# vincentjzy/OpenCorr

Hardware: AMD Instinct MI355X
Metric: converged POIs/sec (FFTCC+ICGN2D1, 33x33 subset) (higher is better)
Workload: dtype f32

## Files before the change

opencorr_amd/csrc/fftcc2d_fused.hip:

```cpp
#include "dic2d_device.h"
#include "fft_device.h"
#include "oc_kernels.h"
#include "host/fftcc_plan.h"

namespace ochip {

namespace {

using namespace fftdev;

constexpr int FN = ochip_host::kFftcc2dFusedSide;
constexpr int FP = FN + 1;
constexpr int FWAVE_LDS = FN * FP;
#ifndef OC_FFTCC2D_X2
#define OC_FFTCC2D_X2 1
#endif
#if !OC_FFTCC2D_X2
#ifndef OC_FFTCC2D_WAVES
#define OC_FFTCC2D_WAVES 4
#endif
constexpr int kFusedWaves = OC_FFTCC2D_WAVES;

template <bool INV>
__device__ __forceinline__ void fft32_line(const c2* line, int step, int h, c2 (&v)[16]) {
#pragma clang fp contract(fast)
    const float sgn = h ? -1.f : 1.f;
#pragma unroll
    for (int n = 0; n < 16; n++) {
        const c2 x0 = line[n * step], x1 = line[(n + 16) * step];
        const c2 d = x0 + sgn * x1;
        const float c = h ? kCos32[n] : 1.f, s = h ? kSin32[n] : 0.f;
        v[n] = (n == 0) ? d : cmul_tw<INV>(d, c, s);
    }
    fft16<INV>(v);
}
#endif

}

#if !OC_FFTCC2D_X2
__global__ __launch_bounds__(64 * kFusedWaves) void fftcc2d_fused32_kernel(Fftcc2dParams P, float* __restrict__ pois,
                                                                           int stride_f, unsigned long long count,
                                                                           int xcd_chunk) {
    __shared__ c2 lds[kFusedWaves * FWAVE_LDS];
    const int lane = threadIdx.x & (kWave - 1);
    const int wave = __builtin_amdgcn_readfirstlane(threadIdx.x >> 6);
    unsigned long long grp = blockIdx.x;
    if (xcd_chunk > 0) grp = (unsigned long long)(blockIdx.x & 7u) * xcd_chunk + (blockIdx.x >> 3);
    const unsigned long long idx = grp * kFusedWaves + wave;
    if (idx >= count) return;
    c2* buf = lds + wave * FWAVE_LDS;
    float* poi = pois + idx * (unsigned long long)stride_f;
    const float px = poi[poi2d::X], py = poi[poi2d::Y];
    const float gu = poi[poi2d::U], gv = poi[poi2d::V];
    const int rx = FN / 2, ry = FN / 2, width = P.width, height = P.height;
    constexpr int M = FN * FN;

    if ((int)px < rx || (int)px >= width - rx || (int)py < ry || (int)py >= height - ry || (int)(px + gu) < rx ||
        (int)(px + gu) >= width - rx || (int)(py + gv) < ry || (int)(py + gv) >= height - ry)
        return;

    float rn, tn;
    {
        const __amdgpu_buffer_rsrc_t r_ref = make_rsrc(P.ref), r_tar = make_rsrc(P.tar);
        float a[16], b[16];
        float rsum = 0.f, tsum = 0.f;
#pragma unroll
        for (int k = 0; k < 16; k++) {
            const int s = lane + kWave * k;
            const int r = s >> 5, c = s & 31;
            const float rxp = px + c - rx, ryp = py + r - ry;
            a[k] = buf_f32(r_ref, (__umul24((unsigned)(int)ryp, (unsigned)width) + (unsigned)(int)rxp) << 2, 0);
            const float txp = rxp + gu, typ = ryp + gv;
            b[k] = buf_f32(r_tar, (__umul24((unsigned)(int)typ, (unsigned)width) + (unsigned)(int)txp) << 2, 0);
        }
#pragma unroll
        for (int k = 0; k < 16; k++) {
            rsum += a[k];
            tsum += b[k];
        }
        const float rmean = wave_allreduce_sum(rsum) / M;
        const float tmean = wave_allreduce_sum(tsum) / M;
        rn = 0.f;
        tn = 0.f;
#pragma unroll
        for (int k = 0; k < 16; k++) {
            const int s = lane + kWave * k;
            const float x = a[k] - rmean, y = b[k] - tmean;
            rn += x * x;
            tn += y * y;
            buf[(s >> 5) * FP + (s & 31)] = mkc(x, y);
        }
        rn = wave_allreduce_sum(rn);
        tn = wave_allreduce_sum(tn);
    }
    __builtin_amdgcn_wave_barrier();

    const int line = lane & 31, h = lane >> 5;
    c2 v[16];
    fft32_line<false>(buf + line * FP, 1, h, v);
    __builtin_amdgcn_wave_barrier();
#pragma unroll
    for (int k = 0; k < 16; k++) buf[line * FP + 2 * k + h] = v[bitrev4(k)];
    __builtin_amdgcn_wave_barrier();
    fft32_line<false>(buf + line, FP, h, v);
    __builtin_amdgcn_wave_barrier();
#pragma unroll
    for (int k = 0; k < 16; k++) buf[(2 * k + h) * FP + line] = v[bitrev4(k)];
    __builtin_amdgcn_wave_barrier();
    {
        const int mx = (FN - line) & (FN - 1);
        c2 zm[16];
#pragma unroll
        for (int k = 0; k < 16; k++) zm[k] = buf[((FN - (2 * k + h)) & (FN - 1)) * FP + mx];
        __builtin_amdgcn_wave_barrier();
#pragma unroll
        for (int k = 0; k < 16; k++) {
            const c2 z = v[bitrev4(k)];
            const float rr = 0.5f * (z.x + zm[k].x), ri = 0.5f * (z.y - zm[k].y);
            const float tr = 0.5f * (z.y + zm[k].y), ti = -0.5f * (z.x - zm[k].x);
            buf[(2 * k + h) * FP + line] = mkc((rr * tr) + (ri * ti), (rr * ti) - (ri * tr));
        }
    }
    __builtin_amdgcn_wave_barrier();
    fft32_line<true>(buf + line * FP, 1, h, v);
    __builtin_amdgcn_wave_barrier();
#pragma unroll
    for (int k = 0; k < 16; k++) buf[line * FP + 2 * k + h] = v[bitrev4(k)];
    __builtin_amdgcn_wave_barrier();
    fft32_line<true>(buf + line, FP, h, v);

    float best = -2.f;
    int bidx = 0;
#pragma unroll
    for (int k = 0; k < 16; k++) {
        const float val = v[bitrev4(k)].x;
        if (val > best) { best = val; bidx = (2 * k + h) * FN + line; }
    }
#pragma unroll
    for (int off = 1; off < kWave; off <<= 1) {
        const float ov = __shfl_xor(best, off, kWave);
        const int oi = __shfl_xor(bidx, off, kWave);
        if (ov > best || (ov == best && oi < bidx)) { best = ov; bidx = oi; }
    }
    if (lane == 0) {
        int du = bidx % FN, dv = bidx / FN;
        if (du > rx) du -= FN;
        if (dv > ry) dv -= FN;
        poi[poi2d::U] = (float)du + gu;
        poi[poi2d::V] = (float)dv + gv;
        poi[poi2d::U0] = gu;
        poi[poi2d::V0] = gv;
        poi[poi2d::ZNCC] = best / (sqrtf(rn * tn) * M);
    }
}
#endif

#ifndef OC_FFTCC2D_X2_WAVES
#define OC_FFTCC2D_X2_WAVES 1
#endif
#ifndef OC_FFTCC2D_X2_SPLIT
#define OC_FFTCC2D_X2_SPLIT 1
#endif
#ifndef OC_FFTCC2D_X2_OCC
#define OC_FFTCC2D_X2_OCC (OC_FFTCC2D_X2_SPLIT ? 4 : 2)
#endif
constexpr int kX2Waves = OC_FFTCC2D_X2_WAVES;

__device__ __forceinline__ float half_wave_sum(float v) {
#pragma unroll
    for (int off = 1; off < 32; off <<= 1) v += __shfl_xor(v, off, kWave);
    return v;
}

template <bool FAST_ROWS, bool REAL_LAST>
__global__ __launch_bounds__(64 * kX2Waves, OC_FFTCC2D_X2_OCC) void fftcc2d_fused32x2_kernel(Fftcc2dParams P, float* __restrict__ pois, int stride_f,
                                                                         unsigned long long count, int xcd_chunk) {
    __shared__ c2 lds[kX2Waves * 2 * FWAVE_LDS / (OC_FFTCC2D_X2_SPLIT ? 2 : 1)];
    const int lane = threadIdx.x & (kWave - 1);
    const int wave = __builtin_amdgcn_readfirstlane(threadIdx.x >> 6);
    const int q = lane >> 5, l = lane & 31;
    unsigned long long grp = blockIdx.x;
    if (xcd_chunk > 0) grp = (unsigned long long)(blockIdx.x & 7u) * xcd_chunk + (blockIdx.x >> 3);
    const unsigned long long idx = (grp * kX2Waves + wave) * 2 + q;
    if (idx >= count) return;
    c2* tile = lds + (wave * 2 + q) * (FWAVE_LDS / (OC_FFTCC2D_X2_SPLIT ? 2 : 1));
    float* poi = pois + idx * (unsigned long long)stride_f;
    const float px = poi[poi2d::X], py = poi[poi2d::Y];
    const float gu = poi[poi2d::U], gv = poi[poi2d::V];
    const int rx = FN / 2, ry = FN / 2, width = P.width, height = P.height;
    constexpr int M = FN * FN;
    if ((int)px < rx || (int)px >= width - rx || (int)py < ry || (int)py >= height - ry || (int)(px + gu) < rx ||
        (int)(px + gu) >= width - rx || (int)(py + gv) < ry || (int)(py + gv) >= height - ry)
        return;

    c2 v[FN];
    float rn, tn;
    {
        const __amdgpu_buffer_rsrc_t r_ref = make_rsrc(P.ref), r_tar = make_rsrc(P.tar);
        const float rxp = px + l - rx, txp = rxp + gu;
        const bool integral = px == (float)(int)px && py == (float)(int)py && gu == (float)(int)gu && gv == (float)(int)gv;
        if (FAST_ROWS && __builtin_amdgcn_ballot_w64(!integral) == 0) {
            const float ry0 = py - ry, ty0 = ry0 + gv;
            const unsigned ref0 = (__umul24((unsigned)(int)ry0, (unsigned)width) + (unsigned)(int)rxp) << 2;
            const unsigned tar0 = (__umul24((unsigned)(int)ty0, (unsigned)width) + (unsigned)(int)txp) << 2;
            const unsigned pitch = (unsigned)width << 2;
#pragma unroll
            for (int k = 0; k < FN; k++) v[k] = mkc(buf_f32(r_ref, ref0, k * pitch), buf_f32(r_tar, tar0, k * pitch));
        } else {
#pragma unroll
            for (int k = 0; k < FN; k++) {
                const float ryp = py + k - ry, typ = ryp + gv;
                const float a = buf_f32(r_ref, (__umul24((unsigned)(int)ryp, (unsigned)width) + (unsigned)(int)rxp) << 2, 0);
                const float b = buf_f32(r_tar, (__umul24((unsigned)(int)typ, (unsigned)width) + (unsigned)(int)txp) << 2, 0);
                v[k] = mkc(a, b);
            }
        }
        float rsum = 0.f, tsum = 0.f;
#pragma unroll
        for (int k = 0; k < FN; k++) {
            rsum += v[k].x;
            tsum += v[k].y;
        }
        const c2 mean = mkc(half_wave_sum(rsum) / M, half_wave_sum(tsum) / M);
        rn = 0.f;
        tn = 0.f;
#pragma unroll
        for (int k = 0; k < FN; k++) {
            v[k] = v[k] - mean;
            rn += v[k].x * v[k].x;
            tn += v[k].y * v[k].y;
        }
        rn = half_wave_sum(rn);
        tn = half_wave_sum(tn);
        asm volatile("" : "+v"(rn), "+v"(tn));
    }
    fft32<false>(v);
#if OC_FFTCC2D_X2_SPLIT
    float* __restrict__ ft = reinterpret_cast<float*>(tile);
#define OC_X2_TRANSPOSE(WRITE_IDX, READ_IDX)                                                   \
    _Pragma("unroll") for (int k = 0; k < FN; k++) ft[WRITE_IDX] = v[bitrev5(k)].x;            \
    __builtin_amdgcn_wave_barrier();                                                           \
    _Pragma("unroll") for (int k = 0; k < FN; k++) v[k].x = ft[READ_IDX];                      \
    __builtin_amdgcn_wave_barrier();                                                           \
    _Pragma("unroll") for (int k = 0; k < FN; k++) ft[WRITE_IDX] = v[bitrev5(k)].y;            \
    __builtin_amdgcn_wave_barrier();                                                           \
    _Pragma("unroll") for (int k = 0; k < FN; k++) v[k].y = ft[READ_IDX];                      \
    __builtin_amdgcn_wave_barrier();
#else
#define OC_X2_TRANSPOSE(WRITE_IDX, READ_IDX)                                                   \
    _Pragma("unroll") for (int k = 0; k < FN; k++) tile[WRITE_IDX] = v[bitrev5(k)];            \
    __builtin_amdgcn_wave_barrier();                                                           \
    _Pragma("unroll") for (int k = 0; k < FN; k++) v[k] = tile[READ_IDX];                      \
    __builtin_amdgcn_wave_barrier();
#endif
    OC_X2_TRANSPOSE(k * FP + l, l * FP + k)
    fft32<false>(v);
    {
        const int mrow = ((FN - l) & (FN - 1)) * FP;
        auto product = [](c2 z, c2 zm) {
            const float rr = z.x + zm.x, ri = z.y - zm.y;
            const float tr = z.y + zm.y, ti = zm.x - z.x;
            return mkc((rr * tr) + (ri * ti), (rr * ti) - (ri * tr));
        };
#if OC_FFTCC2D_X2_SPLIT
        float zmx[FN];
#pragma unroll
        for (int k = 0; k < FN; k++) ft[l * FP + k] = v[bitrev5(k)].x;
        __builtin_amdgcn_wave_barrier();
#pragma unroll
        for (int k = 0; k < FN; k++) zmx[k] = ft[mrow + ((FN - k) & (FN - 1))];
        __builtin_amdgcn_wave_barrier();
#pragma unroll
        for (int k = 0; k < FN; k++) ft[l * FP + k] = v[bitrev5(k)].y;
        __builtin_amdgcn_wave_barrier();
#pragma unroll
        for (int k = 0; k < FN; k++) v[bitrev5(k)] = product(v[bitrev5(k)], mkc(zmx[k], ft[mrow + ((FN - k) & (FN - 1))]));
        __builtin_amdgcn_wave_barrier();
#else
#pragma unroll
        for (int k = 0; k < FN; k++) tile[l * FP + k] = v[bitrev5(k)];
        __builtin_amdgcn_wave_barrier();
#pragma unroll
        for (int k = 0; k < FN; k++) v[bitrev5(k)] = product(v[bitrev5(k)], tile[mrow + ((FN - k) & (FN - 1))]);
        __builtin_amdgcn_wave_barrier();
#endif
    }
    c2 u[FN];
#pragma unroll
    for (int k = 0; k < FN; k++) u[k] = v[bitrev5(k)];
    fft32<true>(u);
#pragma unroll
    for (int k = 0; k < FN; k++) v[k] = u[k];
    float best = -2.f;
    int bidx = 0;
    if constexpr (REAL_LAST) {
#if OC_FFTCC2D_X2_SPLIT
#pragma unroll
        for (int k = 0; k < FN; k++) ft[l * FP + k] = v[bitrev5(k)].x;
        __builtin_amdgcn_wave_barrier();
#pragma unroll
        for (int k = 0; k <= FN / 2; k++) v[k].x = ft[k * FP + l];
        __builtin_amdgcn_wave_barrier();
#pragma unroll
        for (int k = 0; k < FN; k++) ft[l * FP + k] = v[bitrev5(k)].y;
        __builtin_amdgcn_wave_barrier();
#pragma unroll
        for (int k = 0; k <= FN / 2; k++) v[k].y = ft[k * FP + l];
#else
#pragma unroll
        for (int k = 0; k < FN; k++) tile[l * FP + k] = v[bitrev5(k)];
        __builtin_amdgcn_wave_barrier();
#pragma unroll
        for (int k = 0; k <= FN / 2; k++) v[k] = tile[k * FP + l];
#endif
        c2 z[FN / 2];
        ifft32_hermitian(v, z);
        static_for<0, FN>([&](auto rc) {
            constexpr int r = decltype(rc)::value;
            constexpr int pos = fft_pos(FN / 2, r >> 1);
            const float val = (r & 1) ? z[pos].y : z[pos].x;
            if (val > best) { best = val; bidx = r * FN + l; }
        });
    } else {
        OC_X2_TRANSPOSE(l * FP + k, k * FP + l)
#pragma unroll
        for (int k = 0; k < FN; k++) u[k] = v[k];
        fft32<true>(u);
#pragma unroll
        for (int r = 0; r < FN; r++) {
            const float val = u[bitrev5(r)].x;
            if (val > best) { best = val; bidx = r * FN + l; }
        }
    }
#undef OC_X2_TRANSPOSE
#pragma unroll
    for (int off = 1; off < 32; off <<= 1) {
        const float ov = __shfl_xor(best, off, kWave);
        const int oi = __shfl_xor(bidx, off, kWave);
        if (ov > best || (ov == best && oi < bidx)) { best = ov; bidx = oi; }
    }
    if (l == 0) {
        if (rn == 0.f || tn == 0.f) {
            best = 0.f;
            bidx = 0;
        }
        int du = bidx % FN, dv = bidx / FN;
        if (du > rx) du -= FN;
        if (dv > ry) dv -= FN;
        poi[poi2d::U] = (float)du + gu;
        poi[poi2d::V] = (float)dv + gv;
        poi[poi2d::U0] = gu;
        poi[poi2d::V0] = gv;
        poi[poi2d::ZNCC] = (0.25f * best) / (sqrtf(rn * tn) * M);
    }
}

hipError_t launch_fftcc2d_fused(const Fftcc2dParams& p, float* pois, int stride_f, size_t count, bool xcd,
                                hipStream_t stream, int body) {
    if (count == 0) return hipSuccess;
    if (ochip_host::fftcc2d_kernel(p.rx, p.ry, 1) != ochip_host::Fftcc2dKernel::Fused32) return hipErrorInvalidValue;
    (void)hipGetLastError();
#if OC_FFTCC2D_X2
    {
        const size_t groups = (count + 2 * kX2Waves - 1) / (2 * kX2Waves);
        const int chunk = xcd ? (int)((groups + 7) / 8) : 0;
        const size_t grid = xcd ? (size_t)chunk * 8 : groups;
        auto kern = body == 3 ? fftcc2d_fused32x2_kernel<false, false>
                    : body == 4 ? fftcc2d_fused32x2_kernel<true, false>
                    : body == 5 ? fftcc2d_fused32x2_kernel<false, true>
                                : fftcc2d_fused32x2_kernel<true, true>;
        hipLaunchKernelGGL(kern, dim3((unsigned)grid), dim3(64 * kX2Waves), 0, stream, p, pois, stride_f,
                           (unsigned long long)count, chunk);
        return hipGetLastError();
    }
#else
    const size_t groups = (count + kFusedWaves - 1) / kFusedWaves;
    const int chunk = xcd ? (int)((groups + 7) / 8) : 0;
    const size_t grid = xcd ? (size_t)chunk * 8 : groups;
    hipLaunchKernelGGL(fftcc2d_fused32_kernel, dim3((unsigned)grid), dim3(64 * kFusedWaves), 0, stream, p, pois, stride_f,
                       (unsigned long long)count, chunk);
    return hipGetLastError();
#endif
}

}
```

Before: 85.50 million.

## Pair two waves per block to split real-FFT spectrum product work

Adds a paired-wave body for the real-last FFTCC path: two waves (four subsets) share LDS, and one alternating wave computes the Hermitian cross-spectrum product and inverse row FFTs for all four subsets while the other waits. Block size becomes 128 threads for this path and the launch grid is recomputed accordingly. The aim is to halve the redundant product/unpack work and improve balance, at the cost of block-level syncthreads, extra LDS, and idle time for the non-producer wave.

```diff
diff --git a/opencorr_amd/csrc/fftcc2d_fused.hip b/opencorr_amd/csrc/fftcc2d_fused.hip
--- a/opencorr_amd/csrc/fftcc2d_fused.hip
+++ b/opencorr_amd/csrc/fftcc2d_fused.hip
@@ -174,8 +174,8 @@
 }
 
 template <bool FAST_ROWS, bool REAL_LAST>
-__global__ __launch_bounds__(64 * kX2Waves, OC_FFTCC2D_X2_OCC) void fftcc2d_fused32x2_kernel(Fftcc2dParams P, float* __restrict__ pois, int stride_f,
-                                                                         unsigned long long count, int xcd_chunk) {
+__device__ __forceinline__ void fused32x2_wave_body(const Fftcc2dParams& P, float* __restrict__ pois, int stride_f,
+                                                    unsigned long long count, int xcd_chunk) {
     __shared__ c2 lds[kX2Waves * 2 * FWAVE_LDS / (OC_FFTCC2D_X2_SPLIT ? 2 : 1)];
     const int lane = threadIdx.x & (kWave - 1);
     const int wave = __builtin_amdgcn_readfirstlane(threadIdx.x >> 6);
@@ -356,6 +356,239 @@
     }
 }
 
+#ifndef OC_FFTCC2D_X2_PAIR
+#define OC_FFTCC2D_X2_PAIR (OC_FFTCC2D_X2_SPLIT && OC_FFTCC2D_X2_WAVES == 1)
+#endif
+#if OC_FFTCC2D_X2_PAIR
+constexpr int kPairTile = FN * FP + 16;
+constexpr int kPairLds = 4 * kPairTile + 4 * 2 * FN;
+
+template <bool FAST_ROWS>
+__device__ __forceinline__ void fused32x2_pair_body(const Fftcc2dParams& P, float* __restrict__ pois, int stride_f,
+                                                    unsigned long long count, int xcd_chunk) {
+    __shared__ __attribute__((aligned(16))) float lds[kPairLds];
+    const int lane = threadIdx.x & (kWave - 1);
+    const int wave = __builtin_amdgcn_readfirstlane(threadIdx.x >> 6);
+    const int q = lane >> 5, l = lane & 31;
+    unsigned long long grp = blockIdx.x;
+    if (xcd_chunk > 0) grp = (unsigned long long)(blockIdx.x & 7u) * xcd_chunk + (blockIdx.x >> 3);
+    const bool prod = wave == (int)((blockIdx.x >> 3) & 1u);
+    const unsigned long long idx = (grp * 2 + wave) * 2 + q;
+    float* ft = lds + (wave * 2 + q) * kPairTile;
+    float* poi = pois + idx * (unsigned long long)stride_f;
+    const int rx = FN / 2, ry = FN / 2, width = P.width, height = P.height;
+    constexpr int M = FN * FN;
+    float px = 0.f, py = 0.f, gu = 0.f, gv = 0.f;
+    const bool in_queue = idx < count;
+    if (in_queue) {
+        px = poi[poi2d::X];
+        py = poi[poi2d::Y];
+        gu = poi[poi2d::U];
+        gv = poi[poi2d::V];
+    }
+    const bool live = in_queue && !((int)px < rx || (int)px >= width - rx || (int)py < ry || (int)py >= height - ry ||
+                                    (int)(px + gu) < rx || (int)(px + gu) >= width - rx || (int)(py + gv) < ry ||
+                                    (int)(py + gv) >= height - ry);
+    const unsigned long long live_mask = __builtin_amdgcn_ballot_w64(live);
+    auto half_waves = [](float x, float& h0, float& h1) {
+        h0 = __int_as_float(__builtin_amdgcn_readlane(__float_as_int(x), 0));
+        h1 = __int_as_float(__builtin_amdgcn_readlane(__float_as_int(x), 32));
+        asm volatile("" : "+s"(h0), "+s"(h1));
+    };
+    unsigned long long idx0 = (grp * 2 + wave) * 2;
+    asm volatile("" : "+s"(idx0));
+    float gu0, gu1, gv0, gv1, rn0, rn1, tn0, tn1;
+    half_waves(gu, gu0, gu1);
+    half_waves(gv, gv0, gv1);
+
+    c2 v[FN];
+    float rn, tn;
+    {
+        if (!live) {
+            float zero;
+            asm volatile("v_mov_b32 %0, 0" : "=v"(zero));
+#pragma unroll
+            for (int k = 0; k < FN; k++) v[k] = mkc(zero, zero);
+        } else {
+            const __amdgpu_buffer_rsrc_t r_ref = make_rsrc(P.ref), r_tar = make_rsrc(P.tar);
+            const float rxp = px + l - rx, txp = rxp + gu;
+            const bool integral = px == (float)(int)px && py == (float)(int)py && gu == (float)(int)gu && gv == (float)(int)gv;
+            if (FAST_ROWS && __builtin_amdgcn_ballot_w64(!integral) == 0) {
+                const float ry0 = py - ry, ty0 = ry0 + gv;
+                const unsigned ref0 = (__umul24((unsigned)(int)ry0, (unsigned)width) + (unsigned)(int)rxp) << 2;
+                const unsigned tar0 = (__umul24((unsigned)(int)ty0, (unsigned)width) + (unsigned)(int)txp) << 2;
+                const unsigned pitch = (unsigned)width << 2;
+#pragma unroll
+                for (int k = 0; k < FN; k++) v[k] = mkc(buf_f32(r_ref, ref0, k * pitch), buf_f32(r_tar, tar0, k * pitch));
+            } else {
+#pragma unroll
+                for (int k = 0; k < FN; k++) {
+                    const float ryp = py + k - ry, typ = ryp + gv;
+                    const float a = buf_f32(r_ref, (__umul24((unsigned)(int)ryp, (unsigned)width) + (unsigned)(int)rxp) << 2, 0);
+                    const float b = buf_f32(r_tar, (__umul24((unsigned)(int)typ, (unsigned)width) + (unsigned)(int)txp) << 2, 0);
+                    v[k] = mkc(a, b);
+                }
+            }
+        }
+        float rsum = 0.f, tsum = 0.f;
+#pragma unroll
+        for (int k = 0; k < FN; k++) {
+            rsum += v[k].x;
+            tsum += v[k].y;
+        }
+        const c2 mean = mkc(half_wave_sum(rsum) / M, half_wave_sum(tsum) / M);
+        rn = 0.f;
+        tn = 0.f;
+#pragma unroll
+        for (int k = 0; k < FN; k++) {
+            v[k] = v[k] - mean;
+            rn += v[k].x * v[k].x;
+            tn += v[k].y * v[k].y;
+        }
+        half_waves(half_wave_sum(rn), rn0, rn1);
+        half_waves(half_wave_sum(tn), tn0, tn1);
+    }
+    fft32<false>(v);
+#pragma unroll
+    for (int k = 0; k < FN; k++) ft[k * FP + l] = v[bitrev5(k)].x;
+    __builtin_amdgcn_wave_barrier();
+#pragma unroll
+    for (int k = 0; k < FN; k++) v[k].x = ft[l * FP + k];
+    __builtin_amdgcn_wave_barrier();
+#pragma unroll
+    for (int k = 0; k < FN; k++) ft[k * FP + l] = v[bitrev5(k)].y;
+    __builtin_amdgcn_wave_barrier();
+#pragma unroll
+    for (int k = 0; k < FN; k++) v[k].y = ft[l * FP + k];
+    __builtin_amdgcn_wave_barrier();
+    fft32<false>(v);
+
+    const int p = lane >> 4, j = lane & 15;
+    float* pt = lds + p * kPairTile;
+    c2* spare = reinterpret_cast<c2*>(lds + 4 * kPairTile) + p * FN;
+    const int zrow = j * FP, mrow = ((FN - j) & (FN - 1)) * FP;
+    auto product = [](c2 z, c2 zm) {
+        const float rr = z.x + zm.x, ri = z.y - zm.y;
+        const float tr = z.y + zm.y, ti = zm.x - z.x;
+        return mkc((rr * tr) + (ri * ti), (rr * ti) - (ri * tr));
+    };
+    c2 za[FN / 2], zma[FN / 2], ea[4];
+    const int jm = (FN / 2 - j) & (FN / 2 - 1);
+#pragma unroll
+    for (int k = 0; k < FN / 2; k++) {
+        ft[l * FP + 2 * k] = v[bitrev5(k)].x;
+        ft[l * FP + 2 * k + 1] = v[bitrev5(k)].y;
+    }
+#pragma unroll
+    for (int k = FN / 2; k < FN; k++) asm volatile("" : "+v"(v[bitrev5(k)]));
+    __syncthreads();
+    auto at = [&](int row, int k) { return mkc(pt[row + 2 * k], pt[row + 2 * k + 1]); };
+    if (prod) {
+#pragma unroll
+        for (int k = 0; k < FN / 2; k++) {
+            za[k] = at(zrow, k);
+            zma[k] = at(mrow, k);
+        }
+        ea[0] = at(0, j);
+        ea[1] = at((FN / 2) * FP, j);
+        ea[2] = at(0, jm);
+        ea[3] = at((FN / 2) * FP, jm);
+    }
+    __syncthreads();
+#pragma unroll
+    for (int k = 0; k < FN / 2; k++) {
+        ft[l * FP + 2 * k] = v[bitrev5(FN / 2 + k)].x;
+        ft[l * FP + 2 * k + 1] = v[bitrev5(FN / 2 + k)].y;
+    }
+    __syncthreads();
+    if (prod) {
+        c2 u[FN];
+        u[0] = product(za[0], zma[0]);
+        u[FN / 2] = product(at(zrow, 0), at(mrow, 0));
+#pragma unroll
+        for (int k = 1; k < FN / 2; k++) {
+            u[k] = product(za[k], at(mrow, FN / 2 - k));
+            u[FN / 2 + k] = product(at(zrow, k), zma[FN / 2 - k]);
+        }
+        {
+            const c2 eb[4] = {at(0, j), at((FN / 2) * FP, j), at(0, jm), at((FN / 2) * FP, jm)};
+            const bool self = j == 0;
+#pragma unroll
+            for (int t = 0; t < 2; t++) {
+                const c2 z0 = t ? eb[0] : ea[0], z16 = t ? eb[1] : ea[1];
+                const c2 o0 = t ? ea[2] : eb[2], o16 = t ? ea[3] : eb[3];
+                const c2 m0 = mkc(self ? z0.x : o0.x, self ? z0.y : o0.y), m16 = mkc(self ? z16.x : o16.x, self ? z16.y : o16.y);
+                const c2 d0 = product(z0, m0), d16 = product(z16, m16);
+                spare[j + 16 * t] = mkc(d0.x - d16.y, d0.y + d16.x);
+            }
+        }
+        __builtin_amdgcn_wave_barrier();
+        if (j == 0) {
+#pragma unroll
+            for (int k = 0; k < FN; k++) u[k] = spare[k];
+        }
+        fft32<true>(u);
+#pragma unroll
+        for (int c = 0; c < FN; c++) pt[zrow + c] = u[bitrev5(c)].x;
+#pragma unroll
+        for (int c = 0; c < FN; c++) pt[(FN / 2) * FP + zrow + c] = u[bitrev5(c)].y;
+    }
+    __syncthreads();
+
+#pragma unroll
+    for (int k = 0; k <= FN / 2; k++) v[k].x = ft[k * FP + l];
+    v[0].y = 0.f;
+    v[FN / 2].y = 0.f;
+#pragma unroll
+    for (int k = 1; k < FN / 2; k++) v[k].y = ft[(FN / 2 + k) * FP + l];
+    c2 z[FN / 2];
+    ifft32_hermitian(v, z);
+    float best = -2.f;
+    int bidx = 0;
+    static_for<0, FN>([&](auto rc) {
+        constexpr int r = decltype(rc)::value;
+        constexpr int pos = fft_pos(FN / 2, r >> 1);
+        const float val = (r & 1) ? z[pos].y : z[pos].x;
+        if (val > best) { best = val; bidx = r * FN + l; }
+    });
+#pragma unroll
+    for (int off = 1; off < 32; off <<= 1) {
+        const float ov = __shfl_xor(best, off, kWave);
+        const int oi = __shfl_xor(bidx, off, kWave);
+        if (ov > best || (ov == best && oi < bidx)) { best = ov; bidx = oi; }
+    }
+    if (l == 0 && ((live_mask >> lane) & 1ull)) {
+        const float wu = q ? gu1 : gu0, wv = q ? gv1 : gv0, wrn = q ? rn1 : rn0, wtn = q ? tn1 : tn0;
+        float* rec = pois + (idx0 + q) * (unsigned long long)stride_f;
+        if (wrn == 0.f || wtn == 0.f) {
+            best = 0.f;
+            bidx = 0;
+        }
+        int du = bidx % FN, dv = bidx / FN;
+        if (du > rx) du -= FN;
+        if (dv > ry) dv -= FN;
+        rec[poi2d::U] = (float)du + wu;
+        rec[poi2d::V] = (float)dv + wv;
+        rec[poi2d::U0] = wu;
+        rec[poi2d::V0] = wv;
+        rec[poi2d::ZNCC] = (0.25f * best) / (sqrtf(wrn * wtn) * M);
+    }
+}
+#endif
+
+template <bool FAST_ROWS, bool REAL_LAST>
+constexpr int kX2Threads = (REAL_LAST && OC_FFTCC2D_X2_PAIR) ? 128 : 64 * kX2Waves;
+
+template <bool FAST_ROWS, bool REAL_LAST>
+__global__ __launch_bounds__((kX2Threads<FAST_ROWS, REAL_LAST>), OC_FFTCC2D_X2_OCC) void fftcc2d_fused32x2_kernel(
+    Fftcc2dParams P, float* __restrict__ pois, int stride_f, unsigned long long count, int xcd_chunk) {
+#if OC_FFTCC2D_X2_PAIR
+    if constexpr (REAL_LAST) fused32x2_pair_body<FAST_ROWS>(P, pois, stride_f, count, xcd_chunk);
+    else
+#endif
+        fused32x2_wave_body<FAST_ROWS, REAL_LAST>(P, pois, stride_f, count, xcd_chunk);
+}
+
 hipError_t launch_fftcc2d_fused(const Fftcc2dParams& p, float* pois, int stride_f, size_t count, bool xcd,
                                 hipStream_t stream, int body) {
     if (count == 0) return hipSuccess;
@@ -363,14 +596,17 @@
     (void)hipGetLastError();
 #if OC_FFTCC2D_X2
     {
-        const size_t groups = (count + 2 * kX2Waves - 1) / (2 * kX2Waves);
+        const bool real_last = body != 3 && body != 4;
+        const int threads = real_last ? kX2Threads<true, true> : kX2Threads<true, false>;
+        const size_t per_group = (size_t)threads / 32;
+        const size_t groups = (count + per_group - 1) / per_group;
         const int chunk = xcd ? (int)((groups + 7) / 8) : 0;
         const size_t grid = xcd ? (size_t)chunk * 8 : groups;
         auto kern = body == 3 ? fftcc2d_fused32x2_kernel<false, false>
                     : body == 4 ? fftcc2d_fused32x2_kernel<true, false>
                     : body == 5 ? fftcc2d_fused32x2_kernel<false, true>
                                 : fftcc2d_fused32x2_kernel<true, true>;
-        hipLaunchKernelGGL(kern, dim3((unsigned)grid), dim3(64 * kX2Waves), 0, stream, p, pois, stride_f,
+        hipLaunchKernelGGL(kern, dim3((unsigned)grid), dim3(threads), 0, stream, p, pois, stride_f,
                            (unsigned long long)count, chunk);
         return hipGetLastError();
     }
```

New measurement: 86.14 million, median of 6. No clear change (+0.8%).
